# Bluear7878/Remote-Sensing-Vision-Language-Diffusion-Model

Measured on AMD Instinct MI355X. Metric: 512px x8 SR images/sec @50 steps, higher is better.
Workload: dtype f16 / bf16 MFMA operands as hi + lo pairs and triples, f32 accumulation and f32 residual streams (Stage 1: f16 tensors x f16 weight pairs; Stage 2: rsvld_amd.ops.UNET_POLICY; config.precision) -- the composition inside 1e-3 of the reference's CPU path (config.tolerance)

## Files before the change

### remote-sensing-vision-language-diffusion-model_amd/csrc/attention.hip

```cpp
#include "rsvld_common.h"
#include "rsvld_plan.h"
#include <type_traits>
#include <utility>

namespace {

struct AttnArgs {
    const void* q;
    const void* k;
    const void* v;
    void* out;
    int B, heads, Nq, Nk, D;
    int64_t q_bs, q_ts, k_bs, k_ts, v_bs, v_ts, o_bs, o_ts;
    float scale_log2e;
    unsigned long long* dbg;
};

typedef const __attribute__((address_space(1))) void* gptr_t;
typedef __attribute__((address_space(3))) void* lptr_t;

template <typename F, int... I> __device__ __forceinline__ void static_for_impl(F&& f, std::integer_sequence<int, I...>) {
    (f(std::integral_constant<int, I>{}), ...);
}
template <int N, typename F> __device__ __forceinline__ void static_for(F&& f) {
// ... 384 lines not shown
            for (int i = 0; i < NP; ++i) {
                const int rr = 8 * i + (lane >> 3), r16 = (wu * RPW + rr) & 15;
                const int key = min(t * 64 + wu * RPW + rr, p.Nk - 1);
                dma_slow((const char*)(Kb + (int64_t)key * p.k_ts) + (((lane & 7) ^ ((r16 >> 1) & 7)) << 4), kd + i * 1024);
                dma_slow((const char*)(Vb + (int64_t)key * p.v_ts) + (((lane & 7) ^ (((r16 >> 1) & 1) << 2)) << 4), vd + i * 1024);
            }
        }
    };
    dma_tile(0);

    const int qrow = q0 + l31;
    v8 qf[4];
#pragma unroll
    for (int ks = 0; ks < 4; ++ks) {
        u32x4 v = {0u, 0u, 0u, 0u};
        if (qrow < p.Nq) v = *(const u32x4*)(Qb + (int64_t)qrow * p.q_ts + ks * 16 + lh * 8);
        qf[ks] = __builtin_bit_cast(v8, v);
#pragma unroll
        for (int e = 0; e < 8; ++e) qf[ks][e] = (T)((float)qf[ks][e] * p.scale_log2e);
    }
    f32x16 oacc[2];
#pragma unroll
    for (int dt = 0; dt < 2; ++dt)
#pragma unroll
        for (int r = 0; r < 16; ++r) oacc[dt][r] = 0.f;
    float m_run = 0.f, l_run = 0.f;
    uint32_t one_lo;
    {
        T pair[2] = {lh == 0 ? (T)1.f : (T)0.f, (T)0.f};
        __builtin_memcpy(&one_lo, pair, 4);
    }

    int koff[4];
#pragma unroll
    for (int ks = 0; ks < 4; ++ks) koff[ks] = l31 * 128 + (((2 * ks + lh) ^ ((l31 >> 1) & 7)) << 4);
    int voff[2];
    {
        const int qq = (lane >> 2) & 3, pp = lane & 3, g1 = (lane >> 4) & 1;
        const int row = 4 * lh + qq;
#pragma unroll
        for (int dt = 0; dt < 2; ++dt)
            voff[dt] = NB * A6B_TILE + row * 128 + (((4 * dt + 2 * g1 + (pp >> 1)) ^ (((row >> 1) & 1) << 2)) << 4) + ((pp & 1) << 3);
    }

#pragma unroll
    for (int ks = 0; ks < 4; ++ks) asm volatile("" : "+v"(qf[ks]));
    asm volatile("s_waitcnt vmcnt(0)" ::: "memory");
    __syncthreads();

    if (A6B_ABL & 2) {
        if (nt > 1 && KPB == 1) dma_tile(1);
        asm volatile("s_waitcnt vmcnt(0)" ::: "memory");
        __syncthreads();
    }
    v8 abl_frag = *(const v8*)(smem + koff[0]);
    unsigned long long st_sum[5] = {0, 0, 0, 0, 0}, st_t = 0;
    if (A6B_STAMP) st_t = a6b_stamp();
#define A6B_MARK(i) do { if (A6B_STAMP) { const unsigned long long now_ = a6b_stamp(); st_sum[i] += now_ - st_t; st_t = now_; } } while (0)
    for (int t0 = 0; t0 < nt; t0 += KPB) {
    const int t1 = min(t0 + KPB, nt);
#pragma nounroll
    for (int t = t0; t < t1; ++t) {
        const int buf = t & (NB - 1);
        if (A6B_ABL & 48) asm volatile("" : "+v"(abl_frag));
        if (!(A6B_ABL & 2) && t + KPB < nt) dma_tile(t + KPB);
        const char* Ks = smem + buf * A6B_TILE;
        const int vb = buf * A6B_TILE;
        A6B_MARK(0);

        f32x16 sacc[2];
        auto s_phase = [&]() {
        v8 kf[2][4];
        v8 onesf, biasf;
        {
            uint32_t zr;
            asm volatile("v_mov_b32 %0, 0" : "=v"(zr));
            T pair[2] = {(T)(-m_run), (T)0.f};
            uint32_t b0;
            __builtin_memcpy(&b0, pair, 4);
            const u32x4 av = {one_lo, zr, zr, zr}, bv = {b0, zr, zr, zr};
            onesf = __builtin_bit_cast(v8, av);
            biasf = __builtin_bit_cast(v8, bv);
        }
        asm volatile("s_setprio 1");
#pragma unroll
        for (int kt = 0; kt < 2; ++kt) {
#pragma unroll
            for (int ks = 0; ks < 4; ++ks) kf[kt][ks] = (A6B_ABL & 32) ? abl_frag : *(const v8*)(Ks + kt * 4096 + koff[ks]);
            if constexpr (__is_same(T, f16)) {
                asm volatile("s_nop 1\n\tv_mfma_f32_32x32x16_f16 %0, %1, %2, 0" : "=&v"(sacc[kt]) : "v"(onesf), "v"(biasf));
                asm volatile("v_mfma_f32_32x32x16_f16 %0, %1, %2, %0" : "+v"(sacc[kt]) : "v"(kf[kt][0]), "v"(qf[0]));
                asm volatile("v_mfma_f32_32x32x16_f16 %0, %1, %2, %0" : "+v"(sacc[kt]) : "v"(kf[kt][1]), "v"(qf[1]));
                asm volatile("v_mfma_f32_32x32x16_f16 %0, %1, %2, %0" : "+v"(sacc[kt]) : "v"(kf[kt][2]), "v"(qf[2]));
                asm volatile("v_mfma_f32_32x32x16_f16 %0, %1, %2, %0" : "+v"(sacc[kt]) : "v"(kf[kt][3]), "v"(qf[3]));
            } else {
                asm volatile("s_nop 1\n\tv_mfma_f32_32x32x16_bf16 %0, %1, %2, 0" : "=&v"(sacc[kt]) : "v"(onesf), "v"(biasf));
                asm volatile("v_mfma_f32_32x32x16_bf16 %0, %1, %2, %0" : "+v"(sacc[kt]) : "v"(kf[kt][0]), "v"(qf[0]));
                asm volatile("v_mfma_f32_32x32x16_bf16 %0, %1, %2, %0" : "+v"(sacc[kt]) : "v"(kf[kt][1]), "v"(qf[1]));
                asm volatile("v_mfma_f32_32x32x16_bf16 %0, %1, %2, %0" : "+v"(sacc[kt]) : "v"(kf[kt][2]), "v"(qf[2]));
                asm volatile("v_mfma_f32_32x32x16_bf16 %0, %1, %2, %0" : "+v"(sacc[kt]) : "v"(kf[kt][3]), "v"(qf[3]));
            }
        }
        asm volatile("s_setprio 0");
        asm volatile("s_nop 15\n\ts_nop 3" : "+v"(sacc[0]), "+v"(sacc[1]));
        if ((t + 1) * 64 > p.Nk) {
#pragma unroll
            for (int kt = 0; kt < 2; ++kt)
#pragma unroll
                for (int r = 0; r < 16; ++r) {
                    const int kv = t * 64 + kt * 32 + (r & 3) + 8 * (r >> 2) + 4 * lh;
                    if (kv >= p.Nk) sacc[kt][r] = -INFINITY;
                }
        }
        };
        s_phase();
        v8 vf[2][4];
        auto read_v = [&]() {
#pragma unroll
            for (int dt = 0; dt < 2; ++dt)
#pragma unroll
                for (int s4 = 0; s4 < 4; ++s4) {
                    if (A6B_ABL & 16) { vf[dt][s4] = abl_frag; continue; }
                    const int off = vb + voff[dt] + s4 * 2048;
                    const s16x4 lo = __builtin_amdgcn_ds_read_tr16_b64_v4i16((__attribute__((address_space(3))) s16x4*)(smem + off));
                    const s16x4 hi = __builtin_amdgcn_ds_read_tr16_b64_v4i16((__attribute__((address_space(3))) s16x4*)(smem + off + 1024));
                    typedef short s16x8 __attribute__((__vector_size__(8 * sizeof(short))));
                    vf[dt][s4] = __builtin_bit_cast(v8, (s16x8)__builtin_shufflevector(lo, hi, 0, 1, 2, 3, 4, 5, 6, 7));
                }
        };
        A6B_MARK(1);

        float alpha = 1.0f;
        float r4[4] = {0.f, 0.f, 0.f, 0.f};
        auto tile_max = [&]() {
            if (A6B_ABL & 8) return sacc[0][0];
            float m4[4] = {-INFINITY, -INFINITY, -INFINITY, -INFINITY};
#pragma unroll
            for (int kt = 0; kt < 2; ++kt)
#pragma unroll
                for (int r = 0; r < 16; ++r) m4[r >> 2] = fmaxf(m4[r >> 2], sacc[kt][r]);
            return fmaxf(fmaxf(m4[0], m4[1]), fmaxf(m4[2], m4[3]));
        };
        auto exp_and_sum = [&]() {
#pragma unroll
            for (int j = 0; j < 4; ++j) r4[j] = 0.f;
#pragma unroll
            for (int kt = 0; kt < 2; ++kt)
#pragma unroll
                for (int r = 0; r < 16; ++r) {
                    float pv = sacc[kt][r];
                    if (!(A6B_ABL & 1)) pv = __builtin_amdgcn_exp2f(pv);
                    sacc[kt][r] = pv;
                    if (!(A6B_ABL & 8) || r == 0) r4[r >> 2] = a6b_add(r4[r >> 2], pv);
                }
            return a6b_add(a6b_add(r4[0], r4[1]), a6b_add(r4[2], r4[3]));
        };
        float rs = exp_and_sum();
        const bool need = (t == 0) || !(rs <= 16384.0f);
        if (__builtin_expect(__any(need), 0)) {
            s_phase();
            float mx = tile_max();
            {
                const uint32_t mb = __builtin_bit_cast(uint32_t, mx);
                const auto sw = __builtin_amdgcn_permlane32_swap(mb, mb, false, false);
                mx = fmaxf(__builtin_bit_cast(float, (uint32_t)sw[0]), __builtin_bit_cast(float, (uint32_t)sw[1]));
            }
            const bool up = (t == 0) || (mx > 0.0f);
            const float m_new = up ? (float)(T)(m_run + mx) : m_run;
            const float delta = m_new - m_run;
            m_run = m_new;
            alpha = t == 0 ? 1.0f : __builtin_amdgcn_exp2f(-delta);
#pragma unroll
            for (int kt = 0; kt < 2; ++kt)
#pragma unroll
                for (int r = 0; r < 16; ++r) sacc[kt][r] -= delta;
#pragma unroll
            for (int dt = 0; dt < 2; ++dt)
#pragma unroll
                for (int r = 0; r < 16; ++r) oacc[dt][r] *= alpha;
            rs = exp_and_sum();
        }
        l_run = l_run * alpha + rs;
        v8 pf[4];
#pragma unroll
        for (int s4 = 0; s4 < 4; ++s4)
#pragma unroll
            for (int j = 0; j < 8; ++j) pf[s4][j] = (T)sacc[s4 >> 1][8 * (s4 & 1) + j];
        if (A6B_STAMP) {
#pragma unroll
            for (int s4 = 0; s4 < 4; ++s4) asm volatile("" : "+v"(pf[s4]));
            A6B_MARK(2);
        }
        read_v();

        asm volatile("s_setprio 1");
#pragma unroll
        for (int i = 0; i < 8; ++i) {
            const int s4 = i >> 1, dt = i & 1;
            if constexpr (__is_same(T, f16))
                asm volatile("s_nop 1\n\tv_mfma_f32_32x32x16_f16 %0, %1, %2, %0" : "+v"(oacc[dt]) : "v"(vf[dt][s4]), "v"(pf[s4]));
            else
                asm volatile("s_nop 1\n\tv_mfma_f32_32x32x16_bf16 %0, %1, %2, %0" : "+v"(oacc[dt]) : "v"(vf[dt][s4]), "v"(pf[s4]));
        }
        asm volatile("s_setprio 0");
        if (A6B_STAMP) {
            asm volatile("s_nop 15\n\ts_nop 3" : "+v"(oacc[0]), "+v"(oacc[1]));
            A6B_MARK(3);
        }
        asm volatile("s_nop 15\n\ts_nop 3" : "+v"(oacc[0]), "+v"(oacc[1]));
    }
    asm volatile("s_waitcnt vmcnt(0)" ::: "memory");
    if (!(A6B_ABL & 2)) __syncthreads();
    A6B_MARK(4);
    }
    if (A6B_STAMP && p.dbg != nullptr && lane == 0) {
        unsigned long long* d = p.dbg + ((size_t)((blockIdx.z * gridDim.y + blockIdx.y) * gridDim.x + blockIdx.x) * NW + w) * 8;
#pragma unroll
        for (int i = 0; i < 5; ++i) d[i] = st_sum[i];
        d[5] = (unsigned long long)nt;
    }

    const float l_tot = l_run + __shfl_xor(l_run, 32);
    const float inv = 1.0f / l_tot;
    a6_store_o<T>(smem + w * 4096, oacc, inv, q0, lane, p, b, h);
}

#include "attention_d64c.inc"

}

namespace {
struct AttnLaunch {
    AttnArgs a;
    rsvld_plan::AttnPlan pl;
    float *part_o, *part_ml;
    hipStream_t s;
    dim3 grid() const { return dim3((unsigned)pl.grid_x, (unsigned)pl.grid_y, (unsigned)pl.grid_z); }
};
template <auto KERN, int THREADS, int SMEM> int attn_go64(const AttnLaunch& l) {
    if constexpr (SMEM > 0)
        if (rsvld_smem_once<KERN>(SMEM) != hipSuccess) return RSVLD_ELAUNCH;
    hipLaunchKernelGGL(KERN, l.grid(), dim3(THREADS), SMEM, l.s, l.a);
    return rsvld_check_launch();
}
template <auto KERN, auto COMBINE, int SMEM> int attn_go512(const AttnLaunch& l) {
    if (rsvld_smem_once<KERN>(SMEM) != hipSuccess) return RSVLD_ELAUNCH;
    hipLaunchKernelGGL(KERN, l.grid(), dim3(256), SMEM, l.s, l.a, l.pl.keys_per_split, l.part_o, l.part_ml);
    if (l.pl.nsplit > 1)
        hipLaunchKernelGGL(COMBINE, dim3((unsigned)l.a.Nq, (unsigned)(l.a.B * l.a.heads)), dim3(128), 0, l.s, l.a, l.pl.nsplit, l.part_o, l.part_ml);
    return rsvld_check_launch();
}
#define ATTN_ROW64(KERN, THREADS, SMEM) {attn_go64<KERN<f16>, THREADS, SMEM>, attn_go64<KERN<bf16>, THREADS, SMEM>}
#define ATTN_ROW512(SMEM, ...) {attn_go512<__VA_ARGS__<f16>, attn_combine_kernel<f16>, SMEM>, attn_go512<__VA_ARGS__<bf16>, attn_combine_kernel<bf16>, SMEM>}
template <typename T> constexpr auto attn_d64b_nw4 = attn_d64b_kernel<T, 4>;
template <typename T> constexpr auto attn_d64b_nw8 = attn_d64b_kernel<T, 8>;
template <typename T> constexpr auto attn_d512b_two = attn_d512b_kernel<T, false>;
template <typename T> constexpr auto attn_d512b_shared = attn_d512b_kernel<T, true>;
int (*const ATTN_TABLE[6][2])(const AttnLaunch&) = {
    ATTN_ROW64(attn_d64b_nw4, 256, 0),
    ATTN_ROW64(attn_d64b_nw8, 512, 0),
    ATTN_ROW64(attn_d64c_kernel, 512, A6C_SMEM),
    ATTN_ROW512(A5B_SMEM, attn_d512b_two),
    ATTN_ROW512(A5B_SMEM_SH, attn_d512b_shared),
    ATTN_ROW512(A5D_SMEM, attn_d512d_kernel),
};
}

extern "C" int rsvld_plan_attention(int B, int heads, int Nq, int Nk, int D, int plan_div, int tune, int shared_kv, int64_t k_tok_stride,
                                    int64_t v_tok_stride, rsvld_attention_plan* plan) {
    if (plan == nullptr) return RSVLD_EINVAL;
    return rsvld_plan::plan_attention(B, heads, Nq, Nk, D, plan_div, tune, shared_kv != 0, k_tok_stride, v_tok_stride, plan);
}

extern "C" int64_t rsvld_attention_ws_bytes(int B, int heads, int Nq, int Nk, int D, int plan_div) {
    rsvld_plan::AttnPlan pl;
    return rsvld_plan::plan_attention(B, heads, Nq, Nk, D, plan_div, 0, false, 0, 0, &pl) == RSVLD_OK ? pl.ws_bytes : 0;
}

extern "C" int rsvld_attention_tuned(const void* q, const void* k, const void* v, void* out, int B, int heads, int Nq, int Nk,
                                     int D, int64_t q_batch_stride, int64_t q_tok_stride, int64_t k_batch_stride,
                                     int64_t k_tok_stride, int64_t v_batch_stride, int64_t v_tok_stride,
                                     int64_t o_batch_stride, int64_t o_tok_stride, float scale, int dtype, int plan_div,
                                     void* ws, void* stream, int tune) {
    if (!q || !k || !v || !out || B <= 0 || heads <= 0 || Nq <= 0 || Nk <= 0) return RSVLD_EINVAL;
    if (dtype != RSVLD_F16 && dtype != RSVLD_BF16) return RSVLD_EINVAL;
    if ((q_tok_stride | k_tok_stride | v_tok_stride | o_tok_stride | q_batch_stride | k_batch_stride | v_batch_stride |
         o_batch_stride) & 7)
        return RSVLD_EINVAL;
    AttnLaunch l;
    AttnArgs& a = l.a;
    a.q = q; a.k = k; a.v = v; a.out = out;
    a.B = B; a.heads = heads; a.Nq = Nq; a.Nk = Nk; a.D = D;
    a.q_bs = q_batch_stride; a.q_ts = q_tok_stride; a.k_bs = k_batch_stride; a.k_ts = k_tok_stride;
    a.v_bs = v_batch_stride; a.v_ts = v_tok_stride; a.o_bs = o_batch_stride; a.o_ts = o_tok_stride;
    a.scale_log2e = scale * 1.4426950408889634f;
    a.dbg = (A6B_STAMP && D == 64) ? (unsigned long long*)ws : nullptr;
    if (a.dbg != nullptr && tune != RSVLD_ATTN_D64_PINGPONG) tune = RSVLD_ATTN_D64_FOUR_WAVE;
    const bool shared = k == v && k_batch_stride == v_batch_stride && k_tok_stride == v_tok_stride;
    const int rc = rsvld_plan::plan_attention(B, heads, Nq, Nk, D, plan_div, tune, shared, k_tok_stride, v_tok_stride, &l.pl);
    if (rc != RSVLD_OK) return rc;
    if (l.pl.nsplit > 1 && ws == nullptr) return RSVLD_EINVAL;
    l.part_o = (float*)ws;
    l.part_ml = l.pl.nsplit > 1 ? l.part_o + (int64_t)l.pl.nsplit * B * heads * Nq * 512 : nullptr;
    l.s = (hipStream_t)stream;
    return ATTN_TABLE[l.pl.row - 1][dtype == RSVLD_F16 ? 0 : 1](l);
}

extern "C" int rsvld_attention(const void* q, const void* k, const void* v, void* out, int B, int heads, int Nq, int Nk,
                               int D, int64_t q_batch_stride, int64_t q_tok_stride, int64_t k_batch_stride,
                               int64_t k_tok_stride, int64_t v_batch_stride, int64_t v_tok_stride,
                               int64_t o_batch_stride, int64_t o_tok_stride, float scale, int dtype, int plan_div,
                               void* ws, void* stream) {
    return rsvld_attention_tuned(q, k, v, out, B, heads, Nq, Nk, D, q_batch_stride, q_tok_stride, k_batch_stride, k_tok_stride,
                                 v_batch_stride, v_tok_stride, o_batch_stride, o_tok_stride, scale, dtype, plan_div, ws, stream, 0);
}
```

### remote-sensing-vision-language-diffusion-model_amd/csrc/attention_d512d.inc

```
constexpr int A5D_P_OFF = 4 * A5B_TILE;
constexpr int A5D_PBUF = 4 * 2 * 64 * 16;
constexpr int A5D_A_OFF = A5D_P_OFF + 2 * A5D_PBUF;
constexpr int A5D_L_OFF = A5D_A_OFF + 2 * 512;
constexpr int A5D_SMEM = A5D_L_OFF + 512;

template <typename T>
__global__ __launch_bounds__(256) void attn_d512d_kernel(AttnArgs p, int keys_per_split, float* part_o, float* part_ml) {
    constexpr int D = 512;
    typedef typename Mfma<T>::v8 v8;
    typedef typename Mfma<T>::v4 v4;
    extern __shared__ __attribute__((aligned(16))) char smem[];

    const int tid = threadIdx.x, lane = tid & 63, w = tid >> 6;
    const int l31 = lane & 31, lh = lane >> 5;
    const int q0 = blockIdx.x * 128 + w * 32;
    const int split = blockIdx.y, nsplit = gridDim.y;
    const int b = blockIdx.z / p.heads, h = blockIdx.z % p.heads;
    const int k_begin = split * keys_per_split;
    const int k_end = min(p.Nk, k_begin + keys_per_split);
    const int nt = (k_end - k_begin + 31) >> 5;
    const T* Qb = (const T*)p.q + (int64_t)b * p.q_bs + (int64_t)h * D;
    const T* Xb = (const T*)p.k + (int64_t)b * p.k_bs + (int64_t)h * D;

    const int wu = __builtin_amdgcn_readfirstlane(w);
    const uint32_t lds0 = (uint32_t)(uintptr_t)(lptr_t)smem;
    auto dma_one = [&](const char* base, uint32_t voff, uint32_t dst) {
        asm volatile("s_mov_b32 m0, %1\n\ts_nop 0\n\tglobal_load_lds_dwordx4 %0, %2" : : "v"(voff), "s"(dst), "s"(base) : "memory", "m0");
    };
    const int64_t x_rowb = p.k_ts * (int64_t)sizeof(T);
    const uint32_t lane16 = (uint32_t)lane << 4;
    const char* x_tile0 = (const char*)(Xb + (int64_t)(k_begin + wu * 8) * p.k_ts);
    auto dma_x = [&](int t, int i) {
        const int r = wu * 8 + i;
        const uint32_t dst = lds0 + (t & 3) * A5B_TILE + r * 1024;
        if (k_begin + t * 32 + 32 <= p.Nk) {
            dma_one(x_tile0 + (int64_t)(t * 32 + i) * x_rowb, lane16 ^ (uint32_t)(a5b_f(r & 15) << 4), dst);
        } else {
            const int key = min(k_begin + t * 32 + r, p.Nk - 1);
            dma_one((const char*)(Xb + (int64_t)key * p.k_ts), lane16 ^ (uint32_t)(a5b_f(r & 15) << 4), dst);
        }
    };
    auto dma_x_fast = [&](int t, int i) {
        const int r = wu * 8 + i;
        dma_one(x_tile0 + (int64_t)(t * 32 + i) * x_rowb, lane16 ^ (uint32_t)(a5b_f(r & 15) << 4), lds0 + (t & 3) * A5B_TILE + r * 1024);
    };
#pragma unroll
    for (int i = 0; i < 8; ++i) dma_x(0, i);
    if (nt > 1) {
#pragma unroll
        for (int i = 0; i < 8; ++i) dma_x(1, i);
    }
    if (nt > 2) {
#pragma unroll
        for (int i = 0; i < 8; ++i) dma_x(2, i);
    }

    const int qrow = q0 + l31;
    v8 qf[32];
#pragma unroll
    for (int ks = 0; ks < 32; ++ks) {
        u32x4 v = {0u, 0u, 0u, 0u};
        if (qrow < p.Nq) v = *(const u32x4*)(Qb + (int64_t)qrow * p.q_ts + ks * 16 + lh * 8);
        qf[ks] = __builtin_bit_cast(v8, v);
    }
    f32x16 oacc[4][4];
#pragma unroll
    for (int dt = 0; dt < 4; ++dt)
#pragma unroll
        for (int j = 0; j < 4; ++j)
#pragma unroll
            for (int r = 0; r < 16; ++r) oacc[dt][j][r] = 0.f;
    float m_run = -INFINITY, l_run = 0.f;

    const uint32_t kb = l31 * 1024 + ((lh ^ a5b_f(l31 & 15)) << 4);
    int vbase[4];
    {
        const int qq = (lane >> 2) & 3, pp = lane & 3, g1 = (lane >> 4) & 1;
#pragma unroll
        for (int f = 0; f < 4; ++f) vbase[f] = (4 * lh + qq) * 1024 + ((f ^ qq) << 6) + (((2 * g1 + (pp >> 1)) ^ lh) << 4) + ((pp & 1) << 3) + wu * 256;
    }
    auto vread = [&](int buf, int f, int s2) {
        const int off = buf * A5B_TILE + vbase[f] + (16 * s2) * 1024;
        const s16x4 lo = __builtin_amdgcn_ds_read_tr16_b64_v4i16((__attribute__((address_space(3))) s16x4*)(smem + off));
        const s16x4 hi = __builtin_amdgcn_ds_read_tr16_b64_v4i16((__attribute__((address_space(3))) s16x4*)(smem + ((off ^ 32) + 8 * 1024)));
        typedef short s16x8 __attribute__((__vector_size__(8 * sizeof(short))));
        return __builtin_bit_cast(v8, (s16x8)__builtin_shufflevector(lo, hi, 0, 1, 2, 3, 4, 5, 6, 7));
    };
    const int p_own = A5D_P_OFF + wu * 2048 + lane * 16, a_own = A5D_A_OFF + l31 * 16 + wu * 4;
    int p_oth[3], a_oth[3];
#pragma unroll
    for (int j = 1; j < 4; ++j) {
        p_oth[j - 1] = A5D_P_OFF + ((wu + j) & 3) * 2048 + lane * 16;
        a_oth[j - 1] = A5D_A_OFF + l31 * 16 + ((wu + j) & 3) * 4;
    }

    asm volatile("s_waitcnt vmcnt(0)" ::: "memory");
    __syncthreads();

    constexpr int KD = 6;
    uint32_t ka[8];
    v8 kfr[KD];
#define A5D_KREAD(slot, ks) \
    asm volatile("ds_read_b128 %0, %1 offset:%2" : "=v"(kfr[slot]) : "v"(ka[(ks) & 7]), "i"(((ks) >> 3) * 256))
#define A5D_STEP(NAME, SACC, ks)                                                                                        \
    asm volatile("s_waitcnt lgkmcnt(%3)\n\t" NAME " %0, %1, %2, %0"                                                      \
                 : "+v"(SACC)                                                                                           \
                 : "v"(kfr[(ks) % KD]), "v"(qf[ks]), "i"(KD - 1 < 31 - (ks) ? KD - 1 : 31 - (ks)));                      \
    if constexpr ((ks) + KD < 32) A5D_KREAD((ks) % KD, (ks) + KD)
#define A5D_STEP4(NAME, SACC, k) \
    A5D_STEP(NAME, SACC, k); A5D_STEP(NAME, SACC, (k) + 1); A5D_STEP(NAME, SACC, (k) + 2); A5D_STEP(NAME, SACC, (k) + 3)
#define A5D_CHAIN(NAME, SACC, KBUF, HOOK)                                                                               \
    _Pragma("unroll") for (int c = 0; c < 8; ++c) ka[c] = lds0 + (((KBUF) * A5B_TILE + kb) ^ (c << 5));         \
    A5D_KREAD(0, 0); A5D_KREAD(1, 1); A5D_KREAD(2, 2); A5D_KREAD(3, 3); A5D_KREAD(4, 4); A5D_KREAD(5, 5);               \
    asm volatile("s_waitcnt lgkmcnt(%3)\n\t" NAME " %0, %1, %2, 0" : "=&v"(SACC) : "v"(kfr[0]), "v"(qf[0]), "i"(KD - 1)); \
    A5D_KREAD(0, KD);                                                                                                   \
    A5D_STEP(NAME, SACC, 1); A5D_STEP(NAME, SACC, 2); A5D_STEP(NAME, SACC, 3); HOOK(0);                                 \
    A5D_STEP4(NAME, SACC, 4); HOOK(1); A5D_STEP4(NAME, SACC, 8); HOOK(2); A5D_STEP4(NAME, SACC, 12); HOOK(3);           \
    A5D_STEP4(NAME, SACC, 16); HOOK(4); A5D_STEP4(NAME, SACC, 20); HOOK(5); A5D_STEP4(NAME, SACC, 24); HOOK(6);         \
    A5D_STEP4(NAME, SACC, 28); HOOK(7)
#define A5D_NOHOOK(i)

    f32x16 sacc;
    if constexpr (__is_same(T, f16)) {
        A5D_CHAIN("v_mfma_f32_32x32x16_f16", sacc, 0, A5D_NOHOOK);
    } else {
        A5D_CHAIN("v_mfma_f32_32x32x16_bf16", sacc, 0, A5D_NOHOOK);
    }
    asm volatile("s_nop 15\n\ts_nop 3" : "+v"(sacc));

    int t = 0;
    f32x16 sacc2;
#define A5D_STEADY 1
#define A5D_PAIR 1
    for (; t + 5 < nt;) {
        {
#define S_CUR sacc
#define S_NXT sacc2
#include "attention_d512d_body.inc"
#undef S_CUR
#undef S_NXT
        }
        ++t;
        {
#define S_CUR sacc2
#define S_NXT sacc
#include "attention_d512d_body.inc"
#undef S_CUR
#undef S_NXT
        }
        ++t;
    }
#undef A5D_PAIR
#undef A5D_STEADY
    for (; t < nt; ++t) {
#define A5D_PAIR 0
#define A5D_STEADY 0
#define S_CUR sacc
#define S_NXT snext
#include "attention_d512d_body.inc"
#undef S_NXT
#undef S_CUR
#undef A5D_STEADY
#undef A5D_PAIR
    }
#undef A5D_NOHOOK
#undef A5D_CHAIN
#undef A5D_STEP4
#undef A5D_STEP
#undef A5D_KREAD

    const float l_tot = l_run + __shfl_xor(l_run, 32);
    *(float*)(smem + A5D_L_OFF + l31 * 16 + wu * 4) = l_tot;
    __syncthreads();
    float inv[4];
    inv[0] = 1.0f / l_tot;
#pragma unroll
    for (int j = 1; j < 4; ++j) inv[j] = 1.0f / *(const float*)(smem + A5D_L_OFF + l31 * 16 + ((wu + j) & 3) * 4);
#pragma unroll
    for (int j = 0; j < 4; ++j) {
        const int qr = blockIdx.x * 128 + ((wu + j) & 3) * 32 + l31;
        if (qr >= p.Nq) continue;
        if (nsplit == 1) {
            T* Ob = (T*)p.out + (int64_t)b * p.o_bs + (int64_t)h * D + (int64_t)qr * p.o_ts + wu * 128;
#pragma unroll
            for (int dt = 0; dt < 4; ++dt)
#pragma unroll
                for (int g = 0; g < 4; ++g) {
                    v4 o;
#pragma unroll
                    for (int e = 0; e < 4; ++e) o[e] = (T)(oacc[dt][j][4 * g + e] * inv[j]);
                    *(v4*)(Ob + dt * 32 + 8 * g + 4 * lh) = o;
                }
        } else {
            const int64_t row = ((int64_t)split * gridDim.z + blockIdx.z) * p.Nq + qr;
            float* Po = part_o + row * D + wu * 128;
#pragma unroll
            for (int dt = 0; dt < 4; ++dt)
#pragma unroll
                for (int g = 0; g < 4; ++g) {
                    f32x4 o;
#pragma unroll
                    for (int e = 0; e < 4; ++e) o[e] = oacc[dt][j][4 * g + e] * inv[j];
                    *(f32x4*)(Po + dt * 32 + 8 * g + 4 * lh) = o;
                }
            if (j == 0 && lh == 0) {
                part_ml[row * 2] = m_run;
                part_ml[row * 2 + 1] = l_tot;
            }
        }
    }
}
```

### remote-sensing-vision-language-diffusion-model_amd/csrc/attention_d512d_body.inc

```
        const bool more = A5D_STEADY ? true : t + 1 < nt;
        const int b_pv = t & 3, pb = (t & 1) * A5D_PBUF, ab = (t & 1) * 512;

        float mx = -INFINITY, alpha = 1.0f, rs = 0.f;
        bool need = false;
        v8 pf[2];
        auto sm = [&](int part) {
            if (part == 0) {
                if (!A5D_STEADY && k_begin + (t + 1) * 32 > k_end) {
#pragma unroll
                    for (int r = 0; r < 16; ++r) {
                        const int kv = k_begin + t * 32 + (r & 3) + 8 * (r >> 2) + 4 * lh;
                        if (kv >= k_end) S_CUR[r] = -INFINITY;
                    }
                }
#pragma unroll
                for (int r = 0; r < 16; ++r) mx = fmaxf(mx, S_CUR[r]);
                asm volatile("" : "+v"(S_CUR), "+v"(mx));
            } else if (part == 1) {
                mx = a5b_halfwave_max(mx) * p.scale_log2e;
                need = mx > m_run + A5_DEFER_LOG2;
                if (need) {
                    alpha = __builtin_amdgcn_exp2f(m_run - mx);
                    m_run = mx;
                }
                asm volatile("" : "+v"(alpha), "+v"(m_run));
            } else if (part >= 2 && part <= 5) {
                const int r0 = 4 * (part - 2);
#pragma unroll
                for (int r = r0; r < r0 + 4; ++r) {
                    S_CUR[r] = __builtin_amdgcn_exp2f(__builtin_fmaf(S_CUR[r], p.scale_log2e, -m_run));
                    rs += S_CUR[r];
                }
                asm volatile("" : "+v"(S_CUR[r0]), "+v"(S_CUR[r0 + 1]), "+v"(S_CUR[r0 + 2]), "+v"(S_CUR[r0 + 3]), "+v"(rs));
            } else if (part == 6) {
                l_run = l_run * alpha + rs;
#pragma unroll
                for (int s2 = 0; s2 < 2; ++s2)
#pragma unroll
                    for (int j = 0; j < 8; ++j) pf[s2][j] = (T)S_CUR[8 * s2 + j];
                asm volatile("" : "+v"(pf[0]), "+v"(pf[1]), "+v"(l_run));
            }
        };
#if !A5D_PAIR
        f32x16 snext;
#endif
        if (more) {
#define A5D_HOOK(i) \
    sm(i);          \
    __builtin_amdgcn_sched_barrier(0)
            if constexpr (__is_same(T, f16)) {
                A5D_CHAIN("v_mfma_f32_32x32x16_f16", S_NXT, ((t + 1) & 3), A5D_HOOK);
            } else {
                A5D_CHAIN("v_mfma_f32_32x32x16_bf16", S_NXT, ((t + 1) & 3), A5D_HOOK);
            }
#undef A5D_HOOK
        } else {
#pragma unroll
            for (int i = 0; i < 7; ++i) sm(i);
        }

        *(v8*)(smem + pb + p_own) = pf[0];
        *(v8*)(smem + pb + p_own + 1024) = pf[1];
        *(float*)(smem + ab + a_own) = alpha;
        v8 vfr[2][4];
#pragma unroll
        for (int s2 = 0; s2 < 2; ++s2)
#pragma unroll
            for (int f = 0; f < 4; ++f) vfr[s2][f] = vread(b_pv, f, s2);
        asm volatile("s_waitcnt vmcnt(0)" ::: "memory");
        __syncthreads();

        v8 pfo[2][3];
        float al[3];
#pragma unroll
        for (int s2 = 0; s2 < 2; ++s2)
#pragma unroll
            for (int j = 0; j < 3; ++j) pfo[s2][j] = *(const v8*)(smem + pb + p_oth[j] + 1024 * s2);
#pragma unroll
        for (int j = 0; j < 3; ++j) al[j] = *(const float*)(smem + ab + a_oth[j]);

#define A5D_RESCALE(J, A)                                                                                                  \
    _Pragma("unroll") for (int dt = 0; dt < 4; ++dt)                                                                       \
    _Pragma("unroll") for (int r = 0; r < 16; ++r) {                                                                       \
        float x = oacc[dt][J][r], tmp;                                                                                     \
        asm volatile("v_accvgpr_read_b32 %1, %0\n\tv_mul_f32 %1, %1, %2\n\ts_nop 0\n\tv_accvgpr_write_b32 %0, %1\n\ts_nop 1" \
                     : "+a"(x), "=&v"(tmp)                                                                                 \
                     : "v"(A));                                                                                            \
        oacc[dt][J][r] = x;                                                                                                \
    }
        if (__builtin_expect(__any(need), 0)) {
            asm volatile("s_nop 15\n\ts_nop 3" ::: "memory");
            A5D_RESCALE(0, alpha)
        }
        __builtin_amdgcn_sched_barrier(0);
#pragma unroll
        for (int s2 = 0; s2 < 2; ++s2)
#pragma unroll
            for (int f = 0; f < 4; ++f) {
                oacc[f][0] = Mfma<T>::mma(vfr[s2][f], pf[s2], oacc[f][0]);
                __builtin_amdgcn_sched_barrier(0);
            }
        if (__builtin_expect(__any(al[0] != 1.0f || al[1] != 1.0f || al[2] != 1.0f), 0)) {
            asm volatile("s_nop 15\n\ts_nop 3" ::: "memory");
            A5D_RESCALE(1, al[0])
            A5D_RESCALE(2, al[1])
            A5D_RESCALE(3, al[2])
        }
#undef A5D_RESCALE
        __builtin_amdgcn_sched_barrier(0);
#pragma unroll
        for (int n = 0; n < 24; ++n) {
            const int s2 = n / 12, f = (n / 3) & 3, j = n % 3;
            oacc[f][j + 1] = Mfma<T>::mma(vfr[s2][f], pfo[s2][j], oacc[f][j + 1]);
            if (n % 3 == 2) {
                if (A5D_STEADY) {
                    dma_x_fast(t + 3, n / 3);
                } else if (t + 3 < nt) {
                    dma_x(t + 3, n / 3);
                }
            }
            __builtin_amdgcn_sched_barrier(0);
        }
#if !A5D_PAIR
        if (more) S_CUR = S_NXT;
#endif
```

Measured before the change: 0.01402.

## Interleave V/P LDS traffic into QK chain and prefetch next K tile during PV

Moves the P/alpha LDS stores and the V transposed reads into hook slots inside the QK^T MFMA chain, and issues the next tile's K fragment reads (prologue) during the tail of the PV MFMA loop, with relaxed lgkmcnt waits on the last QK steps. It also simplifies LDS address computation (XOR-based vbase, relative peer offsets) to reduce register pressure. Optional timestamp instrumentation is added behind a compile-time flag that defaults off. The goal is to hide LDS latency behind MFMA work, at the cost of tighter scheduling assumptions and more complex waitcnt accounting.

```diff
diff --git a/remote-sensing-vision-language-diffusion-model_amd/csrc/attention.hip b/remote-sensing-vision-language-diffusion-model_amd/csrc/attention.hip
--- a/remote-sensing-vision-language-diffusion-model_amd/csrc/attention.hip
+++ b/remote-sensing-vision-language-diffusion-model_amd/csrc/attention.hip
@@ -710,6 +710,9 @@
     if (l.pl.nsplit > 1 && ws == nullptr) return RSVLD_EINVAL;
     l.part_o = (float*)ws;
     l.part_ml = l.pl.nsplit > 1 ? l.part_o + (int64_t)l.pl.nsplit * B * heads * Nq * 512 : nullptr;
+#if defined(A5D_STAMP) && A5D_STAMP
+    if (D == 512 && ws != nullptr) a.dbg = (unsigned long long*)((char*)ws + l.pl.ws_bytes);
+#endif
     l.s = (hipStream_t)stream;
     return ATTN_TABLE[l.pl.row - 1][dtype == RSVLD_F16 ? 0 : 1](l);
 }
diff --git a/remote-sensing-vision-language-diffusion-model_amd/csrc/attention_d512d.inc b/remote-sensing-vision-language-diffusion-model_amd/csrc/attention_d512d.inc
--- a/remote-sensing-vision-language-diffusion-model_amd/csrc/attention_d512d.inc
+++ b/remote-sensing-vision-language-diffusion-model_amd/csrc/attention_d512d.inc
@@ -4,12 +4,24 @@
 constexpr int A5D_L_OFF = A5D_A_OFF + 2 * 512;
 constexpr int A5D_SMEM = A5D_L_OFF + 512;
 
+#ifndef A5D_STAMP
+#define A5D_STAMP 0
+#endif
+__device__ __forceinline__ unsigned long long a6b_stamp();
+__device__ __forceinline__ unsigned long long a5d_realtime() {
+    unsigned long long t;
+    __builtin_amdgcn_sched_barrier(0);
+    asm volatile("s_memrealtime %0\n\ts_waitcnt lgkmcnt(0)" : "=s"(t) :: "memory");
+    __builtin_amdgcn_sched_barrier(0);
+    return t;
+}
+
 template <typename T>
 __global__ __launch_bounds__(256) void attn_d512d_kernel(AttnArgs p, int keys_per_split, float* part_o, float* part_ml) {
     constexpr int D = 512;
     typedef typename Mfma<T>::v8 v8;
     typedef typename Mfma<T>::v4 v4;
-    extern __shared__ __attribute__((aligned(16))) char smem[];
+    extern __shared__ __attribute__((aligned(1024))) char smem[];
 
     const int tid = threadIdx.x, lane = tid & 63, w = tid >> 6;
     const int l31 = lane & 31, lh = lane >> 5;
@@ -72,27 +84,24 @@
             for (int r = 0; r < 16; ++r) oacc[dt][j][r] = 0.f;
     float m_run = -INFINITY, l_run = 0.f;
 
-    const uint32_t kb = l31 * 1024 + ((lh ^ a5b_f(l31 & 15)) << 4);
-    int vbase[4];
+    const uint32_t kb0 = lds0 + l31 * 1024 + ((lh ^ a5b_f(l31 & 15)) << 4);
+    int vbase0;
     {
         const int qq = (lane >> 2) & 3, pp = lane & 3, g1 = (lane >> 4) & 1;
-#pragma unroll
-        for (int f = 0; f < 4; ++f) vbase[f] = (4 * lh + qq) * 1024 + ((f ^ qq) << 6) + (((2 * g1 + (pp >> 1)) ^ lh) << 4) + ((pp & 1) << 3) + wu * 256;
-    }
-    auto vread = [&](int buf, int f, int s2) {
-        const int off = buf * A5B_TILE + vbase[f] + (16 * s2) * 1024;
+        vbase0 = (4 * lh + qq) * 1024 + (qq << 6) + (((2 * g1 + (pp >> 1)) ^ lh) << 4) + ((pp & 1) << 3) + wu * 256;
+    }
+    auto a5d_keep = [](int x) { asm volatile("" : "+v"(x)); return x; };
+    auto vread = [&](int vb, int buf, int f, int s2) {
+        const int off = buf * A5B_TILE + (vb ^ (f << 6)) + (16 * s2) * 1024;
         const s16x4 lo = __builtin_amdgcn_ds_read_tr16_b64_v4i16((__attribute__((address_space(3))) s16x4*)(smem + off));
         const s16x4 hi = __builtin_amdgcn_ds_read_tr16_b64_v4i16((__attribute__((address_space(3))) s16x4*)(smem + ((off ^ 32) + 8 * 1024)));
         typedef short s16x8 __attribute__((__vector_size__(8 * sizeof(short))));
         return __builtin_bit_cast(v8, (s16x8)__builtin_shufflevector(lo, hi, 0, 1, 2, 3, 4, 5, 6, 7));
     };
     const int p_own = A5D_P_OFF + wu * 2048 + lane * 16, a_own = A5D_A_OFF + l31 * 16 + wu * 4;
-    int p_oth[3], a_oth[3];
-#pragma unroll
-    for (int j = 1; j < 4; ++j) {
-        p_oth[j - 1] = A5D_P_OFF + ((wu + j) & 3) * 2048 + lane * 16;
-        a_oth[j - 1] = A5D_A_OFF + l31 * 16 + ((wu + j) & 3) * 4;
-    }
+    int d_oth[3];
+#pragma unroll
+    for (int j = 1; j < 4; ++j) d_oth[j - 1] = ((wu + j) & 3) - wu;
 
     asm volatile("s_waitcnt vmcnt(0)" ::: "memory");
     __syncthreads();
@@ -107,29 +116,70 @@
                  : "+v"(SACC)                                                                                           \
                  : "v"(kfr[(ks) % KD]), "v"(qf[ks]), "i"(KD - 1 < 31 - (ks) ? KD - 1 : 31 - (ks)));                      \
     if constexpr ((ks) + KD < 32) A5D_KREAD((ks) % KD, (ks) + KD)
+#define A5D_STEPE(NAME, SACC, ks, E)                                                                                    \
+    asm volatile("s_waitcnt lgkmcnt(%3)\n\t" NAME " %0, %1, %2, %0"                                                      \
+                 : "+v"(SACC)                                                                                           \
+                 : "v"(kfr[(ks) % KD]), "v"(qf[ks]), "i"(31 - (ks) + (E) < 15 ? 31 - (ks) + (E) : 15))
 #define A5D_STEP4(NAME, SACC, k) \
     A5D_STEP(NAME, SACC, k); A5D_STEP(NAME, SACC, (k) + 1); A5D_STEP(NAME, SACC, (k) + 2); A5D_STEP(NAME, SACC, (k) + 3)
-#define A5D_CHAIN(NAME, SACC, KBUF, HOOK)                                                                               \
-    _Pragma("unroll") for (int c = 0; c < 8; ++c) ka[c] = lds0 + (((KBUF) * A5B_TILE + kb) ^ (c << 5));         \
-    A5D_KREAD(0, 0); A5D_KREAD(1, 1); A5D_KREAD(2, 2); A5D_KREAD(3, 3); A5D_KREAD(4, 4); A5D_KREAD(5, 5);               \
+#define A5D_KADDR(KBUF, c0, c1) \
+    _Pragma("unroll") for (int c = c0; c < c1; ++c) ka[c] = (kb0 + (KBUF) * A5B_TILE) ^ (c << 5)
+#define A5D_CHAIN_PRO(KBUF) \
+    A5D_KADDR(KBUF, 0, 8);  \
+    A5D_KREAD(0, 0); A5D_KREAD(1, 1); A5D_KREAD(2, 2); A5D_KREAD(3, 3); A5D_KREAD(4, 4); A5D_KREAD(5, 5)
+#define A5D_CHAIN(NAME, SACC, HOOK, E28, E29, E30, E31)                                                                 \
     asm volatile("s_waitcnt lgkmcnt(%3)\n\t" NAME " %0, %1, %2, 0" : "=&v"(SACC) : "v"(kfr[0]), "v"(qf[0]), "i"(KD - 1)); \
     A5D_KREAD(0, KD);                                                                                                   \
+    A5D_MARK(3);                                                                                                        \
     A5D_STEP(NAME, SACC, 1); A5D_STEP(NAME, SACC, 2); A5D_STEP(NAME, SACC, 3); HOOK(0);                                 \
     A5D_STEP4(NAME, SACC, 4); HOOK(1); A5D_STEP4(NAME, SACC, 8); HOOK(2); A5D_STEP4(NAME, SACC, 12); HOOK(3);           \
     A5D_STEP4(NAME, SACC, 16); HOOK(4); A5D_STEP4(NAME, SACC, 20); HOOK(5); A5D_STEP4(NAME, SACC, 24); HOOK(6);         \
-    A5D_STEP4(NAME, SACC, 28); HOOK(7)
+    A5D_STEPE(NAME, SACC, 28, E28); HOOK(8); A5D_STEPE(NAME, SACC, 29, E29); HOOK(9);                                   \
+    A5D_STEPE(NAME, SACC, 30, E30); HOOK(10); A5D_STEPE(NAME, SACC, 31, E31); HOOK(7)
 #define A5D_NOHOOK(i)
+#define A5D_MARK(i)
 
     f32x16 sacc;
+    A5D_CHAIN_PRO(0);
     if constexpr (__is_same(T, f16)) {
-        A5D_CHAIN("v_mfma_f32_32x32x16_f16", sacc, 0, A5D_NOHOOK);
+        A5D_CHAIN("v_mfma_f32_32x32x16_f16", sacc, A5D_NOHOOK, 0, 0, 0, 0);
     } else {
-        A5D_CHAIN("v_mfma_f32_32x32x16_bf16", sacc, 0, A5D_NOHOOK);
+        A5D_CHAIN("v_mfma_f32_32x32x16_bf16", sacc, A5D_NOHOOK, 0, 0, 0, 0);
     }
     asm volatile("s_nop 15\n\ts_nop 3" : "+v"(sacc));
+    if (5 < nt) {
+        A5D_CHAIN_PRO(1);
+    }
+#define A5D_PV_STEP(n)                                                                                                  \
+    {                                                                                                                   \
+        constexpr int s2_ = (n) / 12, f_ = ((n) / 3) & 3, j_ = (n) % 3;                                                 \
+        oacc[f_][j_ + 1] = Mfma<T>::mma(vfr[s2_][f_], pfo[s2_][j_], oacc[f_][j_ + 1]);                                  \
+        if ((n) % 3 == 2) {                                                                                             \
+            if (A5D_STEADY) {                                                                                           \
+                dma_x_fast(t + 3, (n) / 3);                                                                             \
+            } else if (t + 3 < nt) {                                                                                    \
+                dma_x(t + 3, (n) / 3);                                                                                  \
+            }                                                                                                           \
+        }                                                                                                               \
+    }
+#define A5D_PV_TAIL(K)                                                                                                  \
+    A5D_PV_STEP(18); K(0); __builtin_amdgcn_sched_barrier(0); A5D_PV_STEP(19); K(1); __builtin_amdgcn_sched_barrier(0); \
+    A5D_PV_STEP(20); K(2); __builtin_amdgcn_sched_barrier(0); A5D_PV_STEP(21); K(3); __builtin_amdgcn_sched_barrier(0); \
+    A5D_PV_STEP(22); K(4); __builtin_amdgcn_sched_barrier(0); A5D_PV_STEP(23); K(5); __builtin_amdgcn_sched_barrier(0)
+#define A5D_K_NEXT(s) A5D_KREAD(s, s)
+#define A5D_K_NONE(s)
 
     int t = 0;
     f32x16 sacc2;
+#undef A5D_MARK
+    unsigned long long st_sum[4] = {0, 0, 0, 0}, st_t = 0, st_t0 = 0, st_r0 = 0, st_cost = 0;
+#define A5D_MARK(i) do { if (A5D_STAMP == 1) { const unsigned long long now_ = a6b_stamp(); st_sum[i] += now_ - st_t; st_t = now_; } } while (0)
+    if (A5D_STAMP) {
+        st_r0 = a5d_realtime();
+        st_cost = a6b_stamp();
+        st_t0 = st_t = a6b_stamp();
+        st_cost = st_t - st_cost;
+    }
 #define A5D_STEADY 1
 #define A5D_PAIR 1
     for (; t + 5 < nt;) {
@@ -152,6 +202,8 @@
     }
 #undef A5D_PAIR
 #undef A5D_STEADY
+    asm volatile("s_waitcnt lgkmcnt(0)" ::: "memory");
+    __builtin_amdgcn_sched_barrier(0);
     for (; t < nt; ++t) {
 #define A5D_PAIR 0
 #define A5D_STEADY 0
@@ -163,8 +215,23 @@
 #undef A5D_STEADY
 #undef A5D_PAIR
     }
+    if (A5D_STAMP && p.dbg != nullptr && lane == 0) {
+        const unsigned long long t1 = a6b_stamp(), r1 = a5d_realtime();
+        unsigned long long* d = p.dbg + ((size_t)((blockIdx.z * gridDim.y + blockIdx.y) * gridDim.x + blockIdx.x) * 4 + wu) * 8;
+#pragma unroll
+        for (int i = 0; i < 4; ++i) d[i] = st_sum[i];
+        d[4] = t1 - st_t0, d[5] = (unsigned long long)nt, d[6] = r1 - st_r0, d[7] = st_cost;
+    }
+#undef A5D_MARK
+#undef A5D_K_NONE
+#undef A5D_K_NEXT
+#undef A5D_PV_TAIL
+#undef A5D_PV_STEP
 #undef A5D_NOHOOK
 #undef A5D_CHAIN
+#undef A5D_CHAIN_PRO
+#undef A5D_KADDR
+#undef A5D_STEPE
 #undef A5D_STEP4
 #undef A5D_STEP
 #undef A5D_KREAD
diff --git a/remote-sensing-vision-language-diffusion-model_amd/csrc/attention_d512d_body.inc b/remote-sensing-vision-language-diffusion-model_amd/csrc/attention_d512d_body.inc
--- a/remote-sensing-vision-language-diffusion-model_amd/csrc/attention_d512d_body.inc
+++ b/remote-sensing-vision-language-diffusion-model_amd/csrc/attention_d512d_body.inc
@@ -44,40 +44,61 @@
 #if !A5D_PAIR
         f32x16 snext;
 #endif
+        v8 vfr[2][4];
+        const int vb = a5d_keep(vbase0);
+        int pa[3], aa[3];
+        auto lds = [&](int part) {
+            if (part == 10) {
+#pragma unroll
+                for (int j = 0; j < 3; ++j) {
+                    pa[j] = a5d_keep(a5d_keep(p_own) + (pb + d_oth[j] * 2048));
+                    aa[j] = a5d_keep(a5d_keep(a_own) + (ab + d_oth[j] * 4));
+                }
+            }
+            if (part == 6) {
+                *(v8*)(smem + pb + p_own) = pf[0];
+                *(v8*)(smem + pb + p_own + 1024) = pf[1];
+                *(float*)(smem + ab + a_own) = alpha;
+            }
+            if (part == 6 || (part >= 8 && part <= 10)) {
+                const int i = part == 6 ? 0 : part - 7, s2 = i >> 1, f = (i & 1) * 2;
+                vfr[s2][f] = vread(vb, b_pv, f, s2);
+                vfr[s2][f + 1] = vread(vb, b_pv, f + 1, s2);
+            }
+        };
         if (more) {
 #define A5D_HOOK(i) \
     sm(i);          \
+    lds(i);         \
     __builtin_amdgcn_sched_barrier(0)
+#if !A5D_STEADY
+            A5D_CHAIN_PRO((t + 1) & 3);
+#endif
             if constexpr (__is_same(T, f16)) {
-                A5D_CHAIN("v_mfma_f32_32x32x16_f16", S_NXT, ((t + 1) & 3), A5D_HOOK);
+                A5D_CHAIN("v_mfma_f32_32x32x16_f16", S_NXT, A5D_HOOK, 7, 11, 15, 19);
             } else {
-                A5D_CHAIN("v_mfma_f32_32x32x16_bf16", S_NXT, ((t + 1) & 3), A5D_HOOK);
+                A5D_CHAIN("v_mfma_f32_32x32x16_bf16", S_NXT, A5D_HOOK, 7, 11, 15, 19);
             }
 #undef A5D_HOOK
         } else {
+            A5D_MARK(3);
 #pragma unroll
             for (int i = 0; i < 7; ++i) sm(i);
+            lds(6); lds(8); lds(9); lds(10);
         }
-
-        *(v8*)(smem + pb + p_own) = pf[0];
-        *(v8*)(smem + pb + p_own + 1024) = pf[1];
-        *(float*)(smem + ab + a_own) = alpha;
-        v8 vfr[2][4];
-#pragma unroll
-        for (int s2 = 0; s2 < 2; ++s2)
-#pragma unroll
-            for (int f = 0; f < 4; ++f) vfr[s2][f] = vread(b_pv, f, s2);
+        A5D_MARK(0);
         asm volatile("s_waitcnt vmcnt(0)" ::: "memory");
         __syncthreads();
+        A5D_MARK(1);
 
         v8 pfo[2][3];
         float al[3];
 #pragma unroll
         for (int s2 = 0; s2 < 2; ++s2)
 #pragma unroll
-            for (int j = 0; j < 3; ++j) pfo[s2][j] = *(const v8*)(smem + pb + p_oth[j] + 1024 * s2);
+            for (int j = 0; j < 3; ++j) pfo[s2][j] = *(const v8*)(smem + pa[j] + 1024 * s2);
 #pragma unroll
-        for (int j = 0; j < 3; ++j) al[j] = *(const float*)(smem + ab + a_oth[j]);
+        for (int j = 0; j < 3; ++j) al[j] = *(const float*)(smem + aa[j]);
 
 #define A5D_RESCALE(J, A)                                                                                                  \
     _Pragma("unroll") for (int dt = 0; dt < 4; ++dt)                                                                       \
@@ -109,7 +130,7 @@
 #undef A5D_RESCALE
         __builtin_amdgcn_sched_barrier(0);
 #pragma unroll
-        for (int n = 0; n < 24; ++n) {
+        for (int n = 0; n < 18; ++n) {
             const int s2 = n / 12, f = (n / 3) & 3, j = n % 3;
             oacc[f][j + 1] = Mfma<T>::mma(vfr[s2][f], pfo[s2][j], oacc[f][j + 1]);
             if (n % 3 == 2) {
@@ -119,8 +140,16 @@
                     dma_x(t + 3, n / 3);
                 }
             }
+            if (A5D_STEADY && n == 16) { A5D_KADDR((t + 2) & 3, 0, 4); }
+            if (A5D_STEADY && n == 17) { A5D_KADDR((t + 2) & 3, 4, 8); }
             __builtin_amdgcn_sched_barrier(0);
         }
+#if A5D_STEADY
+        A5D_PV_TAIL(A5D_K_NEXT);
+#else
+        A5D_PV_TAIL(A5D_K_NONE);
+#endif
+        A5D_MARK(2);
 #if !A5D_PAIR
         if (more) S_CUR = S_NXT;
 #endif
```

Measured after the change: 0.01403 (median of 2 runs). No clear change (+0.1%).
